# linjieli222/HERO

Hardware: AMD Instinct MI355X
Metric: videos/sec training step, HERO-base TVR-shaped batch (higher is better)
Workload: dtype bf16; 1 GPU; configs[1]: HERO-base TVR finetune micro-step (train-tvr-8gpu.json shapes: 32 videos x 60 frames, 15 subs x (4 frames + 20 tokens), 15-token query; vfeat 4352; fwd + VSM loss + bwd, all-reduce/clip/AdamW every 2nd micro-step); global_batch=32, parallelism=dp1, grad_accum=2, launch=hipGraph replay, input=one batch resident in HBM

## Files before the change

### hero_amd/_lib.py

```python
import ctypes as C
import os

import torch

_HERE = os.path.dirname(os.path.abspath(__file__))
LIB_PATH = os.environ.get("HERO_HIP_LIB") or os.path.join(_HERE, "libhero_hip.so")

ABI_VERSION = 3
F32, BF16 = 0, 1
LAYOUT_K, LAYOUT_O = 0, 1
ACT_NONE, ACT_GELU, ACT_RELU, ACT_GELU_BWD, ACT_RELU_BWD, ACT_GELU_DG, ACT_MUL_AUX = 0, 1, 2, 3, 4, 5, 6

EXPORTS = [
    "hero_last_error", "hero_abi_version", "hero_abi_struct_count", "hero_abi_struct_bytes", "hero_gemm", "hero_gemm_splits", "hero_fold_slabs", "hero_wgrad_group", "hero_wgrad_batch_plan", "hero_wgrad_batch", "hero_prof_enable", "hero_prof_read", "hero_probe_mfma", "hero_probe_hbm", "hero_gemm_force_config", "hero_layernorm_fwd",
    "hero_layernorm_bwd_workspace_bytes", "hero_layernorm_bwd", "hero_colsum_workspace_bytes",
    "hero_colsum", "hero_colsum_multi", "hero_colsum_multi_workspace_bytes", "hero_layernorm_bwd_blocks", "hero_attention_fwd", "hero_attention_bwd", "hero_attention_max_len", "hero_attention_max_packed_len", "hero_attention_stats_ok", "hero_attention_force_ppw",
    "hero_gather_rows", "hero_inverse_first", "hero_csr_gather_sum", "hero_scatter_add_rows", "hero_segment_sort_workspace_bytes", "hero_scatter_add_sorted_workspace_bytes", "hero_segment_sort", "hero_scatter_add_sorted", "hero_cast", "hero_transpose_cast", "hero_copy_multi",
    "hero_relu_bwd", "hero_gelu_bwd", "hero_add", "hero_sumsq", "hero_adamw", "hero_adamw_multi", "hero_adamw_multi_chunk",
    "hero_query_pool_fwd", "hero_query_pool_bwd", "hero_rownorm_fwd", "hero_rownorm_bwd", "hero_score_max_fwd",
    "hero_score_max_bwd", "hero_rank_loss", "hero_sums_scaled", "hero_st_ed_fwd", "hero_st_ed_bwd", "hero_st_ed_bwd_workspace_bytes",
    "hero_cross_entropy_fwd", "hero_cross_entropy_bwd", "hero_qa_pool_fwd", "hero_qa_pool_bwd",
    "hero_topk_rows", "hero_st_ed_probs", "hero_moment_topk", "hero_moment_nms", "hero_first_hit",
    "hero_collate_subs", "hero_collate_clip_mask", "hero_collate_frame_map", "hero_collate_gather_feats", "hero_derive_multi",
    "hero_comm_available", "hero_comm_unique_id", "hero_comm_init", "hero_comm_destroy", "hero_comm_rank", "hero_comm_world",
    "hero_comm_allreduce_buckets", "hero_comm_broadcast", "hero_comm_allgather", "hero_comm_allgather_var",
]


class Dropout(C.Structure):
    _fields_ = [("seed_ptr", C.c_void_p), ("site", C.c_uint64),
                ("threshold16", C.c_uint32), ("scale", C.c_float)]


class GemmEpilogue(C.Structure):
    _fields_ = [("bias", C.c_void_p), ("residual", C.c_void_p), ("aux", C.c_void_p),
                ("act", C.c_int), ("out_f32", C.c_int), ("beta", C.c_float),
                ("split_k", C.c_int), ("dropout", Dropout), ("colsum", C.c_void_p), ("colsum_partial", C.c_int), ("pad_", C.c_int), ("split_stride", C.c_longlong)]
# ... 142 lines not shown
        if have != ABI_VERSION:
            raise RuntimeError("hero_amd: %s reports ABI version %d, this binding was written against %d (struct layouts "
                               "differ: rebuild with `python -m hero_amd.build --force`)" % (LIB_PATH, have, ABI_VERSION))
        L.hero_abi_struct_bytes.argtypes = [C.c_int]
        if L.hero_abi_struct_count() != len(ABI_STRUCTS):
            raise RuntimeError("hero_amd: %s declares %d ABI structs, this binding mirrors %d" % (LIB_PATH, L.hero_abi_struct_count(), len(ABI_STRUCTS)))
        bad = [(st.__name__, C.sizeof(st), L.hero_abi_struct_bytes(i)) for i, st in enumerate(ABI_STRUCTS)
               if C.sizeof(st) != L.hero_abi_struct_bytes(i)]
        if bad:
            raise RuntimeError("hero_amd: struct layouts differ from %s (name, binding bytes, library bytes): %s" % (LIB_PATH, bad))
        L.hero_layernorm_bwd_workspace_bytes.restype = C.c_size_t
        L.hero_colsum_workspace_bytes.restype = C.c_size_t
        L.hero_colsum_multi_workspace_bytes.restype = C.c_size_t
        L.hero_colsum_multi_workspace_bytes.argtypes = [C.POINTER(Colsum), C.c_int]
        L.hero_colsum_multi.argtypes = [C.POINTER(Colsum), C.c_int, C.c_void_p, C.c_void_p]
        L.hero_layernorm_bwd_blocks.argtypes = [C.c_int]
        L.hero_gemm.argtypes = [C.c_void_p, C.c_void_p, C.c_void_p] + [C.c_int] * 9 + [
            C.POINTER(GemmEpilogue), C.c_void_p]
        L.hero_gemm_splits.argtypes = [C.c_int, C.c_int, C.c_int]
        L.hero_fold_slabs.argtypes = [C.c_void_p, C.c_int, C.c_size_t, C.c_void_p, C.c_size_t, C.c_int, C.c_void_p]
        L.hero_wgrad_group.argtypes = [C.POINTER(WgradProblem), C.c_int, C.c_int, C.c_int, C.c_void_p]
        L.hero_wgrad_batch_plan.argtypes = [C.POINTER(WgradProblem), C.c_int, C.c_int, C.c_void_p, C.c_int]
        L.hero_wgrad_batch.argtypes = [C.POINTER(WgradProblem), C.c_int, C.c_int, C.c_int, C.c_void_p, C.c_int, C.c_void_p]
        L.hero_prof_enable.argtypes = [C.c_int]
        L.hero_prof_read.argtypes = [C.c_int, C.POINTER(C.c_double), C.POINTER(C.c_double),
                                     C.POINTER(C.c_longlong)]
        L.hero_probe_mfma.argtypes = [C.c_void_p, C.c_size_t, C.POINTER(C.c_double), C.POINTER(C.c_double), C.c_void_p]
        L.hero_probe_hbm.argtypes = [C.c_void_p, C.c_void_p, C.c_size_t, C.POINTER(C.c_double), C.POINTER(C.c_double), C.c_void_p]
        L.hero_layernorm_fwd.argtypes = [C.POINTER(LnFwd), C.c_void_p]
        L.hero_layernorm_bwd.argtypes = [C.POINTER(LnBwd), C.c_void_p]
        L.hero_layernorm_bwd_workspace_bytes.argtypes = [C.c_int, C.c_int]
        L.hero_colsum_workspace_bytes.argtypes = [C.c_int, C.c_int]
        L.hero_colsum.argtypes = [C.c_void_p, C.c_void_p, C.c_int, C.c_int, C.c_int, C.c_int,
                                  C.c_float, C.c_void_p, C.c_void_p]
        L.hero_attention_fwd.argtypes = [C.POINTER(Attn), C.c_void_p]
        L.hero_attention_bwd.argtypes = [C.POINTER(Attn), C.c_void_p]
        L.hero_attention_stats_ok.argtypes = [C.c_int, C.c_int]
        L.hero_attention_force_ppw.argtypes = [C.c_int]
        L.hero_attention_max_len.argtypes = [C.c_int, C.c_int]
        L.hero_attention_max_packed_len.argtypes = [C.c_int]
        L.hero_gather_rows.argtypes = [C.c_void_p, C.c_void_p, C.c_void_p, C.c_void_p,
                                       C.c_int, C.c_int, C.c_int, C.c_void_p]
        L.hero_inverse_first.argtypes = [C.c_void_p, C.c_int, C.c_void_p, C.c_int, C.c_int, C.c_void_p]
        L.hero_csr_gather_sum.argtypes = [C.c_void_p, C.c_void_p, C.c_void_p, C.c_void_p,
                                          C.c_int, C.c_int, C.c_int, C.c_void_p]
        L.hero_scatter_add_rows.argtypes = [C.c_void_p, C.c_void_p, C.c_void_p, C.c_void_p,
# ... 91 lines not shown
```

### hero_amd/csrc/gemm_ws.hip

```cpp
#include <stdlib.h>
#include <type_traits>

#include "gemm_ws_common.h"

namespace hero {
namespace ws {

template <int TM, int TN, bool TR, int EK>
__global__ __launch_bounds__(512) __attribute__((amdgpu_waves_per_eu(2, 2))) void gemm_ws_kernel(WsArgs g) {
  typedef Geo<TM, TN> G;
  extern __shared__ __attribute__((aligned(16))) char smem[];
  const int lane = threadIdx.x & 63;
  const int wave = __builtin_amdgcn_readfirstlane(threadIdx.x >> 6);
  const int nwg = gridDim.x;
  const int wg = xcd_order(blockIdx.x, nwg);

  if (wave >= 4) {
    Loader<G, TR, ItemSource<G>> ld(ItemSource<G>{g, wg, nwg}, smem, wave - 4, lane);
    constexpr int AHEAD = (G::NSG - 2) * G::PW;
    bool more = ld.issue();
#pragma unroll
    for (int k = 0; k < G::NSG - 2; ++k) more = ld.issue();
    if (more) wait_vm<AHEAD>(); else wait_vm<0>();
    __builtin_amdgcn_s_barrier();
// ... 128 lines not shown
  ml.read_first();
  [[maybe_unused]] int seg_no = 0;
  for (int pos = start; pos < end; ++seg_no) {
    const Seg sg = seg_at<G>(g, pos, end);
    WS_T(seg_no, 0, wave, lane);
    ml.zero<false>();
    ml.run<false>(sg.nk);
    pos += sg.nk;
    WS_T(seg_no, 1, wave, lane);
#ifdef HERO_WS_TRACE
    if (blockIdx.x == 0 && lane == 0 && seg_no < 4) g_ws_trace[(seg_no * 16 + 3) * 8 + wave] = (unsigned long long)sg.nk;
#endif
    const WsgProb& P = g.p[sg.prob];
    atomic_tile<TM, TN>(P.C, P.ldc, P.M, P.N, sg.m0 + wm * TM * 32, sg.n0 + wn * TN * 32, ml.acc, lane);
    WS_T(seg_no, 14, wave, lane);
  }
}

struct WsbProb {
  const bf16_t* A;
  const bf16_t* B;
  float* C;
  float* colsum;
  int M, N, lda, ldb, ldc, pad_;
};
struct WsbItem { int prob, m0, n0, k0, nk, order, nslices, flag; };
struct WsbArgs {
  const WsbItem* items;
  int* flags;
  int rounds, K, nprob, pad_;
  WsbProb p[HERO_WGRAD_BATCH_MAX];
};

template <typename G, bool COMPUTE>
__device__ __forceinline__ void epilogue_acc(const WsbProb& P, const WsbItem& it, int* flags, char* smem, unsigned slot,
                                             f32x16_t (*acc)[G::TN], int wave, int lane, bool want_cs = false) {
  constexpr int BN = G::BN, RPP = G::RPP, RPI = G::RPI, ITERS = G::ITERS;
  char* st = smem + slot;
  const PassLane<G> pl;
  const int tid = pl.tid, c8 = pl.c8, r0 = pl.r0;
  lane = pl.lane;
  wave = pl.wave;
  const int gn = it.n0 + c8 * 8;
  const bool col_ok = r0 < RPI && gn < P.N;
  const bool plain = it.nslices == 1;
  auto tile_row = [](int p, int row) { return PassLane<G>::tile_row(p, row); };
  const __amdgpu_buffer_rsrc_t rc = __builtin_amdgcn_make_buffer_rsrc(P.C, 0, 0x7ffffff0, 0x00020000);
  if (!plain && it.order > 0) {
    if (lane == 0)
      while (__hip_atomic_load(flags + it.flag, __ATOMIC_RELAXED, __HIP_MEMORY_SCOPE_AGENT) != it.order) __builtin_amdgcn_s_sleep(8);
  }
#pragma unroll
  for (int p = 0; p < G::PASSES; ++p) {
    u32x4_t old0[ITERS], old1[ITERS];
// ... 73 lines not shown
    __builtin_amdgcn_s_barrier();
  }
  if (!plain && tid == 0)
    __hip_atomic_store(flags + it.flag, it.order + 1 < it.nslices ? it.order + 1 : 0, __ATOMIC_RELAXED, __HIP_MEMORY_SCOPE_AGENT);
}

__device__ __forceinline__ int wsb_next_round(const WsbArgs& g, int r, int nwg, int wg) {
  while (r < g.rounds && g.items[(size_t)r * nwg + wg].nk == 0) ++r;
  return r;
}

struct PlanSource {
#ifdef HERO_WSB_NOLOADS
  static constexpr bool DMA = false;
#else
  static constexpr bool DMA = true;
#endif
  const WsbArgs& g;
  int nwg, wg, lr;
  __device__ __forceinline__ bool done() const { return lr >= g.rounds; }
  __device__ __forceinline__ Panel panel() const {
    const WsbItem it = g.items[(size_t)lr * nwg + wg];
    const WsbProb& P = g.p[it.prob];
    return Panel{P.A, P.B, P.lda, P.ldb, P.M, P.N, g.K, it.m0, it.n0, it.k0 * 64, it.nk};
  }
  __device__ __forceinline__ void advance() { lr = wsb_next_round(g, lr + 1, nwg, wg); }
};

constexpr int WSB_LAB = 0
#ifdef HERO_WSB_NOLDF
                        | LAB_NOLDF
#endif
#ifdef HERO_WSB_NOMFMA
                        | LAB_NOMFMA
#endif
#ifdef HERO_WSB_NOBAR
                        | LAB_NOBAR
#endif
    ;

__global__ __launch_bounds__(512) __attribute__((amdgpu_waves_per_eu(2, 2))) void gemm_wsb_kernel(WsbArgs g) {
  typedef Geo<3, 3> G;
  constexpr int TM = 3;
  extern __shared__ __attribute__((aligned(16))) char smem[];
  const int lane = threadIdx.x & 63;
  const int wave = __builtin_amdgcn_readfirstlane(threadIdx.x >> 6);
  const int nwg = gridDim.x;
// ... 225 lines not shown
    HERO_ENSURE_LDS(&gemm_wsg_kernel, G::LDS, "gemm_wsg_kernel");
    double flops = 0.0;
    for (int i = 0; i < n; ++i) flops += 2.0 * probs[i].M * (double)probs[i].N * K;
    void* tok = gemm_prof_begin(9, s);
    hipLaunchKernelGGL(gemm_wsg_kernel, dim3(cus), dim3(512), G::LDS, s, g);
    gemm_prof_end(tok, flops, s);
    return check_launch("hero_wgrad_group");
  }
  for (int i = 0; i < n; ++i) {
    const HeroWgradProblem& q = probs[i];
    HeroGemmEpilogue e = {};
    e.out_f32 = 1; e.beta = 1.f; e.split_k = q.split_hint > 0 ? q.split_hint : 1; e.dropout.scale = 1.f;
    const int rc = hero_gemm(q.dy, q.x, q.dw, q.M, q.N, K, q.ld_dy, q.ld_x, q.ld_dw, HERO_LAYOUT_O, HERO_LAYOUT_O, dtype, &e, stream);
    if (rc) return rc;
  }
  return HERO_OK;
}

namespace hero {
namespace ws {
__device__ int g_wsb_flags[512];
constexpr int PLAN_MAGIC = 0x57534232;
constexpr int PLAN_HDR = 8;
}
}

extern "C" int hero_wgrad_batch_plan(const HeroWgradProblem* probs, int n, int K, int32_t* plan, int capacity_words) {
  using namespace hero;
  using namespace hero::ws;
  typedef Geo<3, 3> G;
  HERO_REQUIRE(probs && n >= 1 && n <= HERO_WGRAD_BATCH_MAX, "hero_wgrad_batch_plan: 1..%d problems", HERO_WGRAD_BATCH_MAX);
  HERO_REQUIRE(K >= 1, "hero_wgrad_batch_plan: K = %d", K);
  const int nwg = num_cus(), ksteps = (K + 63) / 64;
  if (nwg % 8 != 0 || ksteps < 8) return 0;
  struct T3 { int prob, mt, nt; };
  std::vector<T3> tiles;
  for (int i = 0; i < n; ++i) {
    HERO_REQUIRE(probs[i].M > 0 && probs[i].N > 0 && probs[i].M % 8 == 0 && probs[i].N % 8 == 0, "hero_wgrad_batch_plan: bad problem %d", i);
    const int tm = (probs[i].M + G::BM - 1) / G::BM, tn = (probs[i].N + G::BN - 1) / G::BN;
    const int per = nwg / 8;
    int pm = tm < 8 ? tm : 8;
    int pn = per / pm > 0 ? per / pm : 1;
    if (pn > tn) { pn = tn; pm = per / pn < tm ? per / pn : tm; if (pm < 1) pm = 1; }
    for (int bm = 0; bm < tm; bm += pm)
      for (int bn = 0; bn < tn; bn += pn)
        for (int mi = bm; mi < bm + pm && mi < tm; ++mi)
          for (int ni = bn; ni < bn + pn && ni < tn; ++ni) tiles.push_back({i, mi, ni});
  }
  const int T = (int)tiles.size();
  const int full = T / nwg, rem = T % nwg;
  struct Piece { int slot, round, tile, k0, nk, order, nslices; };
  std::vector<Piece> pieces;
  int tail_rounds = rem ? 1 : 0, S = 1;
  const int per_xcd_cap = nwg / 8, per_xcd = rem ? (rem + 7) / 8 : 0;
  if (rem) {
    HERO_REQUIRE(per_xcd <= 512 / 8, "hero_wgrad_batch_plan: flag capacity");
    for (int xcd = 0; xcd * per_xcd < rem; ++xcd) {
      const int t0 = xcd * per_xcd, p = (rem - t0 < per_xcd) ? rem - t0 : per_xcd, c = per_xcd_cap;
      int Sx = c / p;
      while (Sx > 1 && ksteps / Sx < 4) --Sx;
      if (Sx > 8) Sx = 8;
      auto cost_us = [&](int sl) { return (double)((ksteps + sl - 1) / sl) * 1.17 + (sl == 1 ? 8.0 : 9.0 + 16.0 * sl); };
      while (Sx > 1 && cost_us(Sx - 1) <= cost_us(Sx)) --Sx;
      const int L = c - Sx * p;
      const int E = 6;
      int q = (int)(((long long)p * ksteps + (long long)(p - L) * E + c - 1) / c);
      int r = ksteps - Sx * q;
      if (L == 0 || Sx != c / p || ksteps < 128 || r * 8 < ksteps) { r = 0; q = ksteps; }
      if (xcd == 0) S = Sx;
      std::vector<std::vector<Piece>> of_tile(p);
      int slot = Sx * p, fillq = 0, rnd = 0;
// ... 14 lines not shown
        }
        int k0 = 0, ord = 0;
        for (int i = (int)mine.size() - 1; i >= 0; --i) { mine[i].k0 = k0; mine[i].order = ord++; k0 += mine[i].nk; }
        of_tile[t] = mine;
      }
      for (int t = 0; t < p; ++t) {
        const int nrem = (int)of_tile[t].size();
        const int big0 = r;
        for (int sl = 0; sl < Sx; ++sl) {
          const int k0 = big0 + (int)((long long)(ksteps - big0) * sl / Sx), k1 = big0 + (int)((long long)(ksteps - big0) * (sl + 1) / Sx);
          of_tile[t].push_back({sl * p + t, 0, t, k0, k1 - k0, nrem + sl, 0});
        }
        for (Piece& pc : of_tile[t]) {
          pc.nslices = (int)of_tile[t].size();
          pc.slot += xcd * per_xcd_cap;
          pc.tile = t0 + t;
          if (pc.round + 1 > tail_rounds) tail_rounds = pc.round + 1;
          pieces.push_back(pc);
        }
      }
    }
  }
  const int rounds = full + tail_rounds;
  const int words = PLAN_HDR + rounds * nwg * 8;
  HERO_REQUIRE(plan && capacity_words >= words, "hero_wgrad_batch_plan: needs %d words, capacity %d", words, capacity_words);
  for (int i = PLAN_HDR; i < words; ++i) plan[i] = 0;
  auto item = [&](int r, int w) { return plan + PLAN_HDR + ((size_t)r * nwg + w) * 8; };
  for (int r = 0; r < full; ++r)
    for (int w = 0; w < nwg; ++w) {
      const T3& t = tiles[(size_t)r * nwg + w];
      int32_t* q = item(r, w);
      q[0] = t.prob; q[1] = t.mt * G::BM; q[2] = t.nt * G::BN; q[3] = 0; q[4] = ksteps; q[5] = 0; q[6] = 1; q[7] = 0;
    }
  for (const Piece& pc : pieces) {
    const T3& t = tiles[(size_t)full * nwg + pc.tile];
    int32_t* q = item(full + pc.round, pc.slot);
    HERO_REQUIRE(q[4] == 0, "hero_wgrad_batch_plan: internal error (slot used twice)");
    q[0] = t.prob; q[1] = t.mt * G::BM; q[2] = t.nt * G::BN; q[3] = pc.k0; q[4] = pc.nk; q[5] = pc.order; q[6] = pc.nslices;
    q[7] = (pc.slot / per_xcd_cap) * (512 / 8) + (pc.tile % per_xcd);
  }
  plan[0] = PLAN_MAGIC; plan[1] = nwg; plan[2] = rounds; plan[3] = rounds * nwg; plan[4] = n; plan[5] = K; plan[6] = T; plan[7] = S;
  return words;
}

extern "C" int hero_wgrad_batch(const HeroWgradProblem* probs, int n, int K, int dtype, const int32_t* plan_dev, int plan_words,
                                hero_stream_t stream) {
  using namespace hero;
  using namespace hero::ws;
  typedef Geo<3, 3> G;
  HERO_REQUIRE(probs && n >= 1 && n <= HERO_WGRAD_BATCH_MAX, "hero_wgrad_batch: 1..%d problems", HERO_WGRAD_BATCH_MAX);
  HERO_REQUIRE(dtype == HERO_BF16, "hero_wgrad_batch: bf16 only (dtype %d)", dtype);
  HERO_REQUIRE(plan_dev && plan_words > PLAN_HDR && (plan_words - PLAN_HDR) % (8 * num_cus()) == 0,
               "hero_wgrad_batch: the plan (%d words) was not made for this device (%d workgroups)", plan_words, num_cus());
  HERO_REQUIRE(((uintptr_t)plan_dev & 15) == 0, "hero_wgrad_batch: plan_dev must be 16-byte aligned");
  hipStream_t s = static_cast<hipStream_t>(stream);
  WsbArgs g;
  double flops = 0.0;
  for (int i = 0; i < n; ++i) {
    const HeroWgradProblem& q = probs[i];
    HERO_REQUIRE(q.dy && q.x && q.dw && q.M > 0 && q.N > 0 && q.M % 8 == 0 && q.N % 8 == 0 && q.ld_dy % 8 == 0 && q.ld_x % 8 == 0 &&
                     q.ld_dw % 4 == 0 && (((uintptr_t)q.dy | (uintptr_t)q.x | (uintptr_t)q.dw) & 15) == 0 &&
                     (size_t)64 * q.ld_dy * 2 < 0x7fffffffull && (size_t)64 * q.ld_x * 2 < 0x7fffffffull &&
                     (size_t)q.M * q.ld_dw * 4 < 0x7ffffff0ull,
                 "hero_wgrad_batch: problem %d is unaligned / too large", i);
    WsbProb& P = g.p[i];
    P.A = static_cast<const bf16_t*>(q.dy); P.B = static_cast<const bf16_t*>(q.x); P.C = q.dw;
    P.M = q.M; P.N = q.N; P.lda = q.ld_dy; P.ldb = q.ld_x; P.ldc = q.ld_dw; P.pad_ = 0;
    P.colsum = q.dbias;
    flops += 2.0 * q.M * (double)q.N * K;
  }
  for (int i = n; i < HERO_WGRAD_BATCH_MAX; ++i) g.p[i] = g.p[0];
  g.items = reinterpret_cast<const WsbItem*>(plan_dev + PLAN_HDR);
  g.rounds = (plan_words - PLAN_HDR) / (8 * num_cus());
  g.K = K; g.nprob = n; g.pad_ = 0;
  static int* flags_of[64] = {};
  int dev = 0;
  (void)hipGetDevice(&dev);
  HERO_REQUIRE(dev >= 0 && dev < 64, "hero_wgrad_batch: device %d", dev);
  if (!flags_of[dev]) HERO_REQUIRE(hipGetSymbolAddress(reinterpret_cast<void**>(&flags_of[dev]), HIP_SYMBOL(hero::ws::g_wsb_flags)) == hipSuccess,
                                   "hero_wgrad_batch: flag storage");
  g.flags = flags_of[dev];
  HERO_ENSURE_LDS(&gemm_wsb_kernel, G::LDS, "gemm_wsb_kernel");
  void* tok = gemm_prof_begin(9, s);
  hipLaunchKernelGGL(gemm_wsb_kernel, dim3(num_cus()), dim3(512), G::LDS, s, g);
  gemm_prof_end(tok, flops, s);
  return check_launch("hero_wgrad_batch");
}
```

### hero_amd/functional.py

```python
import ctypes as C
import math
import os
import weakref

import numpy as np
import torch

from . import _lib as L

_COMPUTE_DTYPE = torch.bfloat16


def set_compute_dtype(dtype):
    global _COMPUTE_DTYPE
    if dtype not in (torch.float32, torch.bfloat16):
        raise ValueError("compute dtype must be torch.float32 or torch.bfloat16")
    _COMPUTE_DTYPE = dtype


def compute_dtype():
    return _COMPUTE_DTYPE


class _Rng:
# ... 302 lines not shown
_WQ_TASK = [-1]
GROUP_WGRADS = [True]
WGRAD_BATCH = [32]
WGRAD_DBIAS_RIDE = [True]
WGRAD_RIDE_MAX_ROWS = [1 << 30]
B1_EPILOGUE = [False]
B1_PARTIALS = [True]
WGRAD_QUEUE_BYTES = [int(os.environ.get("HERO_WGRAD_QUEUE_MB", "4096")) << 20]
_WQ_BYTES = [0]
_WPLANS = {}
_WPLANS_PINNED = set()


def _wgrad_queue_full(device):
    if _WQ_BYTES[0] <= WGRAD_QUEUE_BYTES[0]:
        return False
    hard = _WQ_HARD.get(device.index)
    if hard is None:
        env = os.environ.get("HERO_WGRAD_QUEUE_HARD_MB")
        hard = (int(env) << 20) if env else max(2 * WGRAD_QUEUE_BYTES[0], int(0.15 * torch.cuda.get_device_properties(device).total_memory))
        _WQ_HARD[device.index] = hard
    if _WQ_BYTES[0] > hard:
        return True
    tiles = sum(-(-e[4] // 192) * -(-e[1].shape[1] // 192) for e in _WQ)
    full, rem = divmod(tiles, 256)
    if rem == 0:
        return True
    p = -(-rem // 8)
    slices = max(1, min(32 // p, 8))
    return tiles / 256.0 >= 0.9 * (full + (1.4 if slices > 1 else 1.0) / slices)


_WQ_HARD = {}


def _wgrad_limit():
    return 4 if (WGRAD_BATCH[0] <= 4 or SINK.wants_overlap()) else min(WGRAD_BATCH[0], 32)


def _wgrad_plan(probs, n, rows, device):
    key = (rows, device.index, tuple((probs[i].M, probs[i].N) for i in range(n)))
    hit = _WPLANS.get(key, False)
    if hit is False:
        buf = np.zeros(8 + 8 * 512 * 16, dtype=np.int32)
        words = L.lib().hero_wgrad_batch_plan(probs, n, rows, buf.ctypes.data, buf.size)
        if words < 0:
            L.check(words)
        hit = (torch.from_numpy(buf[:words].copy()).to(device), words) if words > 0 else None
        if len(_WPLANS) > 256:
            for k in [k for k in _WPLANS if k not in _WPLANS_PINNED][:128]:
                del _WPLANS[k]
        _WPLANS[key] = hit
    if hit is not None and torch.cuda.is_current_stream_capturing():
        _WPLANS_PINNED.add(key)
    return hit


_CB_TASK = [-1]


def _ensure_flush_callback(task):
    if _CB_TASK[0] != task:
        _CB_TASK[0] = task
        torch.autograd.Variable._execution_engine.queue_callback(deferred_flush)


def deferred_flush():
    _CB_TASK[0] = -1
# ... 20 lines not shown
        colsum_flush()


def colsum_flush():
    while _CQ:
        part, seen = [], []
        while _CQ and len(part) < 64:
            lo = _CQ[0][1].dst
            hi = lo + 4 * _CQ[0][2].numel()
            if any(lo < b and a < hi for a, b in seen):
                break
            seen.append((lo, hi))
            part.append(_CQ.pop(0))
        n = len(part)
        probs = (L.Colsum * n)(*[e[1] for e in part])
        need = L.lib().hero_colsum_multi_workspace_bytes(probs, n) // 4
        ws = _workspace(max(need, 1), part[0][2].device, slot="colsum_multi")
        L.check(L.lib().hero_colsum_multi(probs, n, L.ptr(ws), L.stream()))
        for e in part:
            if e[3] is not None:
                e[3]()


def wgrad_flush():
    _WQ_BYTES[0] = 0
    while _WQ:
        rows, dtype = _WQ[0][0].shape[0], _WQ[0][0].dtype
        dst_key = lambda e: (e[2].data_ptr(), e[6].data_ptr() if e[6] is not None else None)
        seen_w, seen_b = {_WQ[0][2].data_ptr()}, {dst_key(_WQ[0])[1]} - {None}
        n = 1
        while n < len(_WQ) and n < 32 and _WQ[n][0].shape[0] == rows and _WQ[n][0].dtype == dtype:
            kw, kb = dst_key(_WQ[n])
            if kw in seen_w or (kb is not None and kb in seen_b):
                break
            seen_w.add(kw)
            if kb is not None:
                seen_b.add(kb)
            n += 1
        group, rest = _WQ[:n], _WQ[n:]
        del _WQ[:]
        _WQ.extend(rest)
        probs = (L.WgradProblem * n)()
        for i, (dy2, x2, out, col0, N, _, _, _) in enumerate(group):
            K = x2.shape[1]
            probs[i] = L.WgradProblem(L.ptr(dy2) + col0 * dy2.element_size(), L.ptr(x2), L.ptr(out), N, K,
                                      dy2.shape[1], K, K, _split_for(N, K, rows, 64 if dtype == torch.bfloat16 else 32), None)
        plan = _wgrad_plan(probs, n, rows, group[0][0].device) if dtype == torch.bfloat16 else None
        if plan is not None:
            ride = WGRAD_DBIAS_RIDE[0] and rows <= WGRAD_RIDE_MAX_ROWS[0]
            for i, e in enumerate(group):
                probs[i].dbias = L.ptr(e[6]) if ride else None
                if not ride and e[6] is not None:
                    k_colsum(e[0], out=e[6], beta=1.0, col0=e[3], ncols=e[4], on_done=lambda: None)
            L.check(L.lib().hero_wgrad_batch(probs, n, rows, L.BF16, L.ptr(plan[0]), plan[1], L.stream()))
            for e in group:
                if e[6] is not None and e[7] is not None:
                    e[7]()
        else:
            for g0 in range(0, n, 4):
                sub = (L.WgradProblem * min(4, n - g0))(*[probs[i] for i in range(g0, min(g0 + 4, n))])
                L.check(L.lib().hero_wgrad_group(sub, len(sub), rows, L.dt(group[0][0]), L.stream()))
            for dy2, _, _, col0, N, _, dbias, dbias_done in group:
                if dbias is not None:
                    k_colsum(dy2, out=dbias, beta=1.0, col0=col0, ncols=N, on_done=dbias_done or (lambda: None))
        for e in group:
            if e[5] is not None:
                e[5]()


def k_wgrad(dy2, x2, out=None, beta=0.0, col0=0, ncols=None, on_done=None, dbias=None, dbias_done=None):
    M, ld = dy2.shape
    N = ld - col0 if ncols is None else ncols
    K = x2.shape[1]
    if (out is not None and beta == 1.0 and GROUP_WGRADS[0] and out.is_contiguous() and dy2.is_contiguous()
            and x2.is_contiguous() and torch._C._current_graph_task_id() != -1):
        task = torch._C._current_graph_task_id()
        if _WQ and _WQ_TASK[0] != task:
            del _WQ[:]
            _WQ_BYTES[0] = 0
        if _WQ and (_WQ[0][0].shape[0] != M or _WQ[0][0].dtype != dy2.dtype):
            wgrad_flush()
        if not _WQ:
            _WQ_TASK[0] = task
        _ensure_flush_callback(task)
        _WQ.append((dy2, x2, out, col0, N, on_done, dbias, dbias_done))
        _WQ_BYTES[0] += dy2.numel() * dy2.element_size()
        if len(_WQ) >= _wgrad_limit() or _wgrad_queue_full(dy2.device):
            wgrad_flush()
        return out
    if dbias is not None:
        k_colsum(dy2, out=dbias, beta=1.0, col0=col0, ncols=N, on_done=dbias_done or (lambda: None))
    if out is None:
        out = torch.empty((N, K), dtype=torch.float32, device=dy2.device)
    split = _split_for(N, K, M, 64 if dy2.dtype == torch.bfloat16 else 32)
    a = L.ptr(dy2) + col0 * dy2.element_size()
    k_gemm(a, x2, out, N, K, M, ld, K, K, L.LAYOUT_O, L.LAYOUT_O, L.dt(dy2), out_f32=True,
           beta=beta, split_k=split)
    if on_done is not None:
        on_done()
    return out


_WS = {}


def _workspace(n_floats, device, slot=""):
    key = (device.type, device.index, slot)
    t = _WS.get(key)
    if t is None or t.numel() < n_floats:
        t = torch.empty((max(n_floats, 1 << 20),), dtype=torch.float32, device=device)
# ... 916 lines not shown
```

### include/hero_hip.h

```cpp
#ifndef HERO_HIP_H_
#define HERO_HIP_H_

#include <stddef.h>
#include <stdint.h>

#ifdef __cplusplus
extern "C" {
#endif

typedef void* hero_stream_t;

enum { HERO_F32 = 0, HERO_BF16 = 1 };
enum { HERO_OK = 0, HERO_ERR_ARG = -1, HERO_ERR_LAUNCH = -2, HERO_ERR_UNSUPPORTED = -3 };

const char* hero_last_error(void);
#define HERO_ABI_VERSION 3
int hero_abi_version(void);
enum { HERO_STRUCT_DROPOUT = 0, HERO_STRUCT_GEMM_EPILOGUE, HERO_STRUCT_WGRAD_PROBLEM, HERO_STRUCT_LN_FWD, HERO_STRUCT_LN_BWD,
       HERO_STRUCT_COLSUM, HERO_STRUCT_ATTN, HERO_STRUCT_ADAMW, HERO_STRUCT_TENSOR_DESC, HERO_STRUCT_ADAMW_GROUP,
       HERO_STRUCT_ADAMW_MULTI, HERO_STRUCT_COPY_DESC, HERO_STRUCT_QUERY_POOL, HERO_STRUCT_ROW_NORM, HERO_STRUCT_SCORE_MAX,
       HERO_STRUCT_RANK_LOSS, HERO_STRUCT_ST_ED, HERO_STRUCT_CROSS_ENTROPY, HERO_STRUCT_DERIVE, HERO_STRUCT_COMM_BUCKET,
       HERO_STRUCT_COUNT_ };
int hero_abi_struct_count(void);
int hero_abi_struct_bytes(int which);
// ... 28 lines not shown
  int colsum_partial;
  int pad_;
  long long split_stride;
} HeroGemmEpilogue;

int hero_gemm(const void* A, const void* B, void* C, int M, int N, int K, int lda, int ldb, int ldc,
              int a_layout, int b_layout, int dtype, const HeroGemmEpilogue* epi, hero_stream_t stream);
int hero_gemm_splits(int K, int split_k, int dtype);
int hero_fold_slabs(const float* slabs, int n_slabs, size_t stride, void* out, size_t n, int out_dtype, hero_stream_t stream);

typedef struct HeroWgradProblem {
  const void* dy;
  const void* x;
  float* dw;
  int M, N, ld_dy, ld_x, ld_dw;
  int split_hint;
  float* dbias;
} HeroWgradProblem;
int hero_wgrad_group(const HeroWgradProblem* probs, int n, int K, int dtype, hero_stream_t stream);
#define HERO_WGRAD_BATCH_MAX 32
int hero_wgrad_batch_plan(const HeroWgradProblem* probs, int n, int K, int32_t* plan, int capacity_words);
int hero_wgrad_batch(const HeroWgradProblem* probs, int n, int K, int dtype, const int32_t* plan_dev, int plan_words,
                     hero_stream_t stream);
int hero_gemm_force_config(int cfg);
int hero_prof_enable(int on);
int hero_prof_read(int slot, double* total_ms, double* total_flops, long long* launches);

int hero_probe_mfma(void* scratch, size_t scratch_bytes, double* tflops, double* ghz, hero_stream_t stream);
int hero_probe_hbm(const void* src, void* dst, size_t bytes, double* copy_gbps, double* read_gbps, hero_stream_t stream);

typedef struct HeroLnFwd {
  const void* x;
  const float* tab[3];
  const int32_t* idx[3];
  const float* gamma;
  const float* beta;
  void* y;
  void* pre;
  float* mean;
  float* rstd;
  int rows, cols;
  float eps;
  int x_dtype, y_dtype;
  HeroDropout dropout;
} HeroLnFwd;
int hero_layernorm_fwd(const HeroLnFwd* a, hero_stream_t stream);
// ... 295 lines not shown
```

Baseline: 5524 videos/s.

## Batch weight-gradient GEMMs with different row counts into one persistent launch

Extends the persistent batched wgrad kernel so each problem carries its own reduction length K. The planner schedules the longest-K problems with the existing equal-split scheme, then greedily places shorter-K tiles onto the least-loaded workgroups, favouring whichever XCD has the most such workgroups. The Python queue no longer flushes when the row count changes, so wgrads from different encoders (e.g. frame and token paths) can share one launch of up to 64 problems. This reduces launch count and tail idle time, but brings a larger kernel argument struct, more complex host planning, and a changed flush heuristic that may form groups of different sizes.

```diff
diff --git a/hero_amd/_lib.py b/hero_amd/_lib.py
--- a/hero_amd/_lib.py
+++ b/hero_amd/_lib.py
@@ -12,7 +12,7 @@
 ACT_NONE, ACT_GELU, ACT_RELU, ACT_GELU_BWD, ACT_RELU_BWD, ACT_GELU_DG, ACT_MUL_AUX = 0, 1, 2, 3, 4, 5, 6
 
 EXPORTS = [
-    "hero_last_error", "hero_abi_version", "hero_abi_struct_count", "hero_abi_struct_bytes", "hero_gemm", "hero_gemm_splits", "hero_fold_slabs", "hero_wgrad_group", "hero_wgrad_batch_plan", "hero_wgrad_batch", "hero_prof_enable", "hero_prof_read", "hero_probe_mfma", "hero_probe_hbm", "hero_gemm_force_config", "hero_layernorm_fwd",
+    "hero_last_error", "hero_abi_version", "hero_abi_struct_count", "hero_abi_struct_bytes", "hero_gemm", "hero_gemm_splits", "hero_fold_slabs", "hero_wgrad_group", "hero_wgrad_batch_plan", "hero_wgrad_batch", "hero_wgrad_batch_plan_rows", "hero_wgrad_batch_rows", "hero_prof_enable", "hero_prof_read", "hero_probe_mfma", "hero_probe_hbm", "hero_gemm_force_config", "hero_layernorm_fwd",
     "hero_layernorm_bwd_workspace_bytes", "hero_layernorm_bwd", "hero_colsum_workspace_bytes",
     "hero_colsum", "hero_colsum_multi", "hero_colsum_multi_workspace_bytes", "hero_layernorm_bwd_blocks", "hero_attention_fwd", "hero_attention_bwd", "hero_attention_max_len", "hero_attention_max_packed_len", "hero_attention_stats_ok", "hero_attention_force_ppw",
     "hero_gather_rows", "hero_inverse_first", "hero_csr_gather_sum", "hero_scatter_add_rows", "hero_segment_sort_workspace_bytes", "hero_scatter_add_sorted_workspace_bytes", "hero_segment_sort", "hero_scatter_add_sorted", "hero_cast", "hero_transpose_cast", "hero_copy_multi",
@@ -201,6 +201,8 @@
         L.hero_wgrad_group.argtypes = [C.POINTER(WgradProblem), C.c_int, C.c_int, C.c_int, C.c_void_p]
         L.hero_wgrad_batch_plan.argtypes = [C.POINTER(WgradProblem), C.c_int, C.c_int, C.c_void_p, C.c_int]
         L.hero_wgrad_batch.argtypes = [C.POINTER(WgradProblem), C.c_int, C.c_int, C.c_int, C.c_void_p, C.c_int, C.c_void_p]
+        L.hero_wgrad_batch_plan_rows.argtypes = [C.POINTER(WgradProblem), C.c_int, C.POINTER(C.c_int), C.c_void_p, C.c_int]
+        L.hero_wgrad_batch_rows.argtypes = [C.POINTER(WgradProblem), C.c_int, C.POINTER(C.c_int), C.c_int, C.c_void_p, C.c_int, C.c_void_p]
         L.hero_prof_enable.argtypes = [C.c_int]
         L.hero_prof_read.argtypes = [C.c_int, C.POINTER(C.c_double), C.POINTER(C.c_double),
                                      C.POINTER(C.c_longlong)]
diff --git a/hero_amd/csrc/gemm_ws.hip b/hero_amd/csrc/gemm_ws.hip
--- a/hero_amd/csrc/gemm_ws.hip
+++ b/hero_amd/csrc/gemm_ws.hip
@@ -174,14 +174,15 @@
   const bf16_t* B;
   float* C;
   float* colsum;
-  int M, N, lda, ldb, ldc, pad_;
+  int M, N, lda, ldb, ldc;
+  int K;
 };
 struct WsbItem { int prob, m0, n0, k0, nk, order, nslices, flag; };
 struct WsbArgs {
   const WsbItem* items;
   int* flags;
-  int rounds, K, nprob, pad_;
-  WsbProb p[HERO_WGRAD_BATCH_MAX];
+  int rounds, nprob, pad_[2];
+  WsbProb p[HERO_WGRAD_BATCH_ROWS_MAX];
 };
 
 template <typename G, bool COMPUTE>
@@ -301,7 +302,7 @@
   __device__ __forceinline__ Panel panel() const {
     const WsbItem it = g.items[(size_t)lr * nwg + wg];
     const WsbProb& P = g.p[it.prob];
-    return Panel{P.A, P.B, P.lda, P.ldb, P.M, P.N, g.K, it.m0, it.n0, it.k0 * 64, it.nk};
+    return Panel{P.A, P.B, P.lda, P.ldb, P.M, P.N, P.K, it.m0, it.n0, it.k0 * 64, it.nk};
   }
   __device__ __forceinline__ void advance() { lr = wsb_next_round(g, lr + 1, nwg, wg); }
 };
@@ -573,31 +574,27 @@
 __device__ int g_wsb_flags[512];
 constexpr int PLAN_MAGIC = 0x57534232;
 constexpr int PLAN_HDR = 8;
-}
-}
-
-extern "C" int hero_wgrad_batch_plan(const HeroWgradProblem* probs, int n, int K, int32_t* plan, int capacity_words) {
-  using namespace hero;
-  using namespace hero::ws;
+
+struct T3 { int prob, mt, nt; };
+
+static void patch_tiles(const HeroWgradProblem& q, int prob, int nwg, std::vector<T3>& tiles) {
   typedef Geo<3, 3> G;
-  HERO_REQUIRE(probs && n >= 1 && n <= HERO_WGRAD_BATCH_MAX, "hero_wgrad_batch_plan: 1..%d problems", HERO_WGRAD_BATCH_MAX);
-  HERO_REQUIRE(K >= 1, "hero_wgrad_batch_plan: K = %d", K);
-  const int nwg = num_cus(), ksteps = (K + 63) / 64;
-  if (nwg % 8 != 0 || ksteps < 8) return 0;
-  struct T3 { int prob, mt, nt; };
+  const int tm = (q.M + G::BM - 1) / G::BM, tn = (q.N + G::BN - 1) / G::BN;
+  const int per = nwg / 8;
+  int pm = tm < 8 ? tm : 8;
+  int pn = per / pm > 0 ? per / pm : 1;
+  if (pn > tn) { pn = tn; pm = per / pn < tm ? per / pn : tm; if (pm < 1) pm = 1; }
+  for (int bm = 0; bm < tm; bm += pm)
+    for (int bn = 0; bn < tn; bn += pn)
+      for (int mi = bm; mi < bm + pm && mi < tm; ++mi)
+        for (int ni = bn; ni < bn + pn && ni < tn; ++ni) tiles.push_back({prob, mi, ni});
+}
+
+static int plan_equal(const HeroWgradProblem* probs, const int* idx, int m, int K, int nwg, std::vector<int32_t>& items, int* T_out, int* S_out) {
+  typedef Geo<3, 3> G;
+  const int ksteps = (K + 63) / 64;
   std::vector<T3> tiles;
-  for (int i = 0; i < n; ++i) {
-    HERO_REQUIRE(probs[i].M > 0 && probs[i].N > 0 && probs[i].M % 8 == 0 && probs[i].N % 8 == 0, "hero_wgrad_batch_plan: bad problem %d", i);
-    const int tm = (probs[i].M + G::BM - 1) / G::BM, tn = (probs[i].N + G::BN - 1) / G::BN;
-    const int per = nwg / 8;
-    int pm = tm < 8 ? tm : 8;
-    int pn = per / pm > 0 ? per / pm : 1;
-    if (pn > tn) { pn = tn; pm = per / pn < tm ? per / pn : tm; if (pm < 1) pm = 1; }
-    for (int bm = 0; bm < tm; bm += pm)
-      for (int bn = 0; bn < tn; bn += pn)
-        for (int mi = bm; mi < bm + pm && mi < tm; ++mi)
-          for (int ni = bn; ni < bn + pn && ni < tn; ++ni) tiles.push_back({i, mi, ni});
-  }
+  for (int j = 0; j < m; ++j) patch_tiles(probs[idx[j]], idx[j], nwg, tiles);
   const int T = (int)tiles.size();
   const int full = T / nwg, rem = T % nwg;
   struct Piece { int slot, round, tile, k0, nk, order, nslices; };
@@ -658,10 +655,8 @@
     }
   }
   const int rounds = full + tail_rounds;
-  const int words = PLAN_HDR + rounds * nwg * 8;
-  HERO_REQUIRE(plan && capacity_words >= words, "hero_wgrad_batch_plan: needs %d words, capacity %d", words, capacity_words);
-  for (int i = PLAN_HDR; i < words; ++i) plan[i] = 0;
-  auto item = [&](int r, int w) { return plan + PLAN_HDR + ((size_t)r * nwg + w) * 8; };
+  items.assign((size_t)rounds * nwg * 8, 0);
+  auto item = [&](int r, int w) { return items.data() + ((size_t)r * nwg + w) * 8; };
   for (int r = 0; r < full; ++r)
     for (int w = 0; w < nwg; ++w) {
       const T3& t = tiles[(size_t)r * nwg + w];
@@ -675,50 +670,147 @@
     q[0] = t.prob; q[1] = t.mt * G::BM; q[2] = t.nt * G::BN; q[3] = pc.k0; q[4] = pc.nk; q[5] = pc.order; q[6] = pc.nslices;
     q[7] = (pc.slot / per_xcd_cap) * (512 / 8) + (pc.tile % per_xcd);
   }
-  plan[0] = PLAN_MAGIC; plan[1] = nwg; plan[2] = rounds; plan[3] = rounds * nwg; plan[4] = n; plan[5] = K; plan[6] = T; plan[7] = S;
+  *T_out = T; *S_out = S;
+  return rounds;
+}
+
+static int plan_rows(const HeroWgradProblem* probs, int n, const int* rows, int nwg, int32_t* plan, int capacity_words, const char* who) {
+  typedef Geo<3, 3> G;
+  HERO_REQUIRE(probs && rows && n >= 1 && n <= HERO_WGRAD_BATCH_ROWS_MAX, "%s: 1..%d problems", who, HERO_WGRAD_BATCH_ROWS_MAX);
+  HERO_REQUIRE(nwg >= 1, "%s: %d workgroups", who, nwg);
+  int kmax = 0;
+  for (int i = 0; i < n; ++i) {
+    HERO_REQUIRE(rows[i] >= 1, "%s: K = %d (problem %d)", who, rows[i], i);
+    if (rows[i] > kmax) kmax = rows[i];
+  }
+  if (nwg % 8 != 0 || (kmax + 63) / 64 < 8) return 0;
+  for (int i = 0; i < n; ++i)
+    HERO_REQUIRE(probs[i].M > 0 && probs[i].N > 0 && probs[i].M % 8 == 0 && probs[i].N % 8 == 0, "%s: bad problem %d", who, i);
+  std::vector<int> idx;
+  for (int i = 0; i < n; ++i)
+    if (rows[i] == kmax) idx.push_back(i);
+  std::vector<int32_t> items;
+  int T = 0, S = 1;
+  int rounds = plan_equal(probs, idx.data(), (int)idx.size(), kmax, nwg, items, &T, &S);
+  if (rounds < 0) return rounds;
+  if ((int)idx.size() < n) {
+    const int c = nwg / 8;
+    std::vector<long long> load(nwg, 0);
+    std::vector<int> next(nwg, 0);
+    for (int r = 0; r < rounds; ++r)
+      for (int w = 0; w < nwg; ++w) {
+        const int nk = items[((size_t)r * nwg + w) * 8 + 4];
+        if (nk) { load[w] += nk; next[w] = r + 1; }
+      }
+    int below = kmax;
+    for (;;) {
+      int K = 0;
+      for (int i = 0; i < n; ++i)
+        if (rows[i] < below && rows[i] > K) K = rows[i];
+      if (K == 0) break;
+      below = K;
+      const int ksteps = (K + 63) / 64;
+      std::vector<T3> tiles;
+      for (int i = 0; i < n; ++i)
+        if (rows[i] == K) patch_tiles(probs[i], i, nwg, tiles);
+      T += (int)tiles.size();
+      for (size_t t0 = 0; t0 < tiles.size();) {
+        int wmin = 0;
+        for (int w = 1; w < nwg; ++w)
+          if (load[w] < load[wmin]) wmin = w;
+        int best = -1, best_cnt = 0;
+        for (int x = 0; x < 8; ++x) {
+          int cnt = 0;
+          for (int w = x * c; w < (x + 1) * c; ++w) cnt += load[w] == load[wmin];
+          if (cnt > best_cnt) { best = x; best_cnt = cnt; }
+        }
+        const long long lv = load[wmin];
+        for (int w = best * c; w < (best + 1) * c && t0 < tiles.size(); ++w) {
+          if (load[w] != lv) continue;
+          if (next[w] == rounds) { ++rounds; items.resize((size_t)rounds * nwg * 8, 0); }
+          const T3& t = tiles[t0++];
+          int32_t* q = items.data() + ((size_t)next[w] * nwg + w) * 8;
+          HERO_REQUIRE(q[4] == 0, "%s: internal error (slot used twice)", who);
+          q[0] = t.prob; q[1] = t.mt * G::BM; q[2] = t.nt * G::BN; q[3] = 0; q[4] = ksteps; q[5] = 0; q[6] = 1; q[7] = 0;
+          load[w] += ksteps; ++next[w];
+        }
+      }
+    }
+  }
+  const int words = PLAN_HDR + rounds * nwg * 8;
+  HERO_REQUIRE(plan && capacity_words >= words, "%s: needs %d words, capacity %d", who, words, capacity_words);
+  for (int i = PLAN_HDR; i < words; ++i) plan[i] = items[i - PLAN_HDR];
+  plan[0] = PLAN_MAGIC; plan[1] = nwg; plan[2] = rounds; plan[3] = rounds * nwg; plan[4] = n; plan[5] = kmax; plan[6] = T; plan[7] = S;
   return words;
 }
 
-extern "C" int hero_wgrad_batch(const HeroWgradProblem* probs, int n, int K, int dtype, const int32_t* plan_dev, int plan_words,
-                                hero_stream_t stream) {
-  using namespace hero;
-  using namespace hero::ws;
+static int launch_rows(const HeroWgradProblem* probs, int n, const int* rows, int dtype, const int32_t* plan_dev, int plan_words,
+                       hero_stream_t stream, const char* who) {
   typedef Geo<3, 3> G;
-  HERO_REQUIRE(probs && n >= 1 && n <= HERO_WGRAD_BATCH_MAX, "hero_wgrad_batch: 1..%d problems", HERO_WGRAD_BATCH_MAX);
-  HERO_REQUIRE(dtype == HERO_BF16, "hero_wgrad_batch: bf16 only (dtype %d)", dtype);
+  HERO_REQUIRE(probs && rows && n >= 1 && n <= HERO_WGRAD_BATCH_ROWS_MAX, "%s: 1..%d problems", who, HERO_WGRAD_BATCH_ROWS_MAX);
+  HERO_REQUIRE(dtype == HERO_BF16, "%s: bf16 only (dtype %d)", who, dtype);
   HERO_REQUIRE(plan_dev && plan_words > PLAN_HDR && (plan_words - PLAN_HDR) % (8 * num_cus()) == 0,
-               "hero_wgrad_batch: the plan (%d words) was not made for this device (%d workgroups)", plan_words, num_cus());
-  HERO_REQUIRE(((uintptr_t)plan_dev & 15) == 0, "hero_wgrad_batch: plan_dev must be 16-byte aligned");
+               "%s: the plan (%d words) was not made for this device (%d workgroups)", who, plan_words, num_cus());
+  HERO_REQUIRE(((uintptr_t)plan_dev & 15) == 0, "%s: plan_dev must be 16-byte aligned", who);
   hipStream_t s = static_cast<hipStream_t>(stream);
   WsbArgs g;
   double flops = 0.0;
   for (int i = 0; i < n; ++i) {
     const HeroWgradProblem& q = probs[i];
+    HERO_REQUIRE(rows[i] >= 1, "%s: K = %d (problem %d)", who, rows[i], i);
     HERO_REQUIRE(q.dy && q.x && q.dw && q.M > 0 && q.N > 0 && q.M % 8 == 0 && q.N % 8 == 0 && q.ld_dy % 8 == 0 && q.ld_x % 8 == 0 &&
                      q.ld_dw % 4 == 0 && (((uintptr_t)q.dy | (uintptr_t)q.x | (uintptr_t)q.dw) & 15) == 0 &&
                      (size_t)64 * q.ld_dy * 2 < 0x7fffffffull && (size_t)64 * q.ld_x * 2 < 0x7fffffffull &&
                      (size_t)q.M * q.ld_dw * 4 < 0x7ffffff0ull,
-                 "hero_wgrad_batch: problem %d is unaligned / too large", i);
+                 "%s: problem %d is unaligned / too large", who, i);
     WsbProb& P = g.p[i];
     P.A = static_cast<const bf16_t*>(q.dy); P.B = static_cast<const bf16_t*>(q.x); P.C = q.dw;
-    P.M = q.M; P.N = q.N; P.lda = q.ld_dy; P.ldb = q.ld_x; P.ldc = q.ld_dw; P.pad_ = 0;
+    P.M = q.M; P.N = q.N; P.lda = q.ld_dy; P.ldb = q.ld_x; P.ldc = q.ld_dw; P.K = rows[i];
     P.colsum = q.dbias;
-    flops += 2.0 * q.M * (double)q.N * K;
-  }
-  for (int i = n; i < HERO_WGRAD_BATCH_MAX; ++i) g.p[i] = g.p[0];
+    flops += 2.0 * q.M * (double)q.N * rows[i];
+  }
+  for (int i = n; i < HERO_WGRAD_BATCH_ROWS_MAX; ++i) g.p[i] = g.p[0];
   g.items = reinterpret_cast<const WsbItem*>(plan_dev + PLAN_HDR);
   g.rounds = (plan_words - PLAN_HDR) / (8 * num_cus());
-  g.K = K; g.nprob = n; g.pad_ = 0;
+  g.nprob = n; g.pad_[0] = g.pad_[1] = 0;
   static int* flags_of[64] = {};
   int dev = 0;
   (void)hipGetDevice(&dev);
-  HERO_REQUIRE(dev >= 0 && dev < 64, "hero_wgrad_batch: device %d", dev);
+  HERO_REQUIRE(dev >= 0 && dev < 64, "%s: device %d", who, dev);
   if (!flags_of[dev]) HERO_REQUIRE(hipGetSymbolAddress(reinterpret_cast<void**>(&flags_of[dev]), HIP_SYMBOL(hero::ws::g_wsb_flags)) == hipSuccess,
-                                   "hero_wgrad_batch: flag storage");
+                                   "%s: flag storage", who);
   g.flags = flags_of[dev];
   HERO_ENSURE_LDS(&gemm_wsb_kernel, G::LDS, "gemm_wsb_kernel");
   void* tok = gemm_prof_begin(9, s);
   hipLaunchKernelGGL(gemm_wsb_kernel, dim3(num_cus()), dim3(512), G::LDS, s, g);
   gemm_prof_end(tok, flops, s);
-  return check_launch("hero_wgrad_batch");
-}
+  return check_launch(who);
+}
+}
+}
+
+extern "C" int hero_wgrad_batch_plan_rows(const HeroWgradProblem* probs, int n, const int* rows, int32_t* plan, int capacity_words) {
+  return hero::ws::plan_rows(probs, n, rows, hero::num_cus(), plan, capacity_words, "hero_wgrad_batch_plan_rows");
+}
+
+extern "C" int hero_wgrad_batch_plan(const HeroWgradProblem* probs, int n, int K, int32_t* plan, int capacity_words) {
+  using namespace hero;
+  HERO_REQUIRE(probs && n >= 1 && n <= HERO_WGRAD_BATCH_MAX, "hero_wgrad_batch_plan: 1..%d problems", HERO_WGRAD_BATCH_MAX);
+  int rows[HERO_WGRAD_BATCH_MAX];
+  for (int i = 0; i < n; ++i) rows[i] = K;
+  return ws::plan_rows(probs, n, rows, num_cus(), plan, capacity_words, "hero_wgrad_batch_plan");
+}
+
+extern "C" int hero_wgrad_batch_rows(const HeroWgradProblem* probs, int n, const int* rows, int dtype, const int32_t* plan_dev,
+                                     int plan_words, hero_stream_t stream) {
+  return hero::ws::launch_rows(probs, n, rows, dtype, plan_dev, plan_words, stream, "hero_wgrad_batch_rows");
+}
+
+extern "C" int hero_wgrad_batch(const HeroWgradProblem* probs, int n, int K, int dtype, const int32_t* plan_dev, int plan_words,
+                                hero_stream_t stream) {
+  using namespace hero;
+  HERO_REQUIRE(probs && n >= 1 && n <= HERO_WGRAD_BATCH_MAX, "hero_wgrad_batch: 1..%d problems", HERO_WGRAD_BATCH_MAX);
+  int rows[HERO_WGRAD_BATCH_MAX];
+  for (int i = 0; i < n; ++i) rows[i] = K;
+  return ws::launch_rows(probs, n, rows, dtype, plan_dev, plan_words, stream, "hero_wgrad_batch");
+}
diff --git a/hero_amd/functional.py b/hero_amd/functional.py
--- a/hero_amd/functional.py
+++ b/hero_amd/functional.py
@@ -348,13 +348,15 @@
         _WQ_HARD[device.index] = hard
     if _WQ_BYTES[0] > hard:
         return True
-    tiles = sum(-(-e[4] // 192) * -(-e[1].shape[1] // 192) for e in _WQ)
+    kmax = max(e[1].shape[0] for e in _WQ)
+    tiles = sum(-(-e[4] // 192) * -(-e[1].shape[1] // 192) for e in _WQ if e[1].shape[0] == kmax)
+    short = sum(-(-e[4] // 192) * -(-e[1].shape[1] // 192) * -(-e[1].shape[0] // 64) for e in _WQ if e[1].shape[0] != kmax) / float(-(-kmax // 64))
     full, rem = divmod(tiles, 256)
     if rem == 0:
         return True
     p = -(-rem // 8)
     slices = max(1, min(32 // p, 8))
-    return tiles / 256.0 >= 0.9 * (full + (1.4 if slices > 1 else 1.0) / slices)
+    return (tiles + short) / 256.0 >= 0.9 * (full + (1.4 if slices > 1 else 1.0) / slices + short / 256.0)
 
 
 _WQ_HARD = {}
@@ -364,12 +366,21 @@
     return 4 if (WGRAD_BATCH[0] <= 4 or SINK.wants_overlap()) else min(WGRAD_BATCH[0], 32)
 
 
+WGRAD_LAUNCH_MAX = 64
+
+
+def _wgrad_count_full(rows):
+    lim = _wgrad_limit()
+    return sum(1 for e in _WQ if e[1].shape[0] == rows) >= lim or len(_WQ) >= max(lim, WGRAD_LAUNCH_MAX)
+
+
 def _wgrad_plan(probs, n, rows, device):
+    rows = (rows,) * n if isinstance(rows, int) else tuple(rows)
     key = (rows, device.index, tuple((probs[i].M, probs[i].N) for i in range(n)))
     hit = _WPLANS.get(key, False)
     if hit is False:
         buf = np.zeros(8 + 8 * 512 * 16, dtype=np.int32)
-        words = L.lib().hero_wgrad_batch_plan(probs, n, rows, buf.ctypes.data, buf.size)
+        words = L.lib().hero_wgrad_batch_plan_rows(probs, n, (C.c_int * n)(*rows), buf.ctypes.data, buf.size)
         if words < 0:
             L.check(words)
         hit = (torch.from_numpy(buf[:words].copy()).to(device), words) if words > 0 else None
@@ -436,44 +447,58 @@
                 e[3]()
 
 
+def _wgrad_take(same_rows):
+    rows, dtype = _WQ[0][0].shape[0], _WQ[0][0].dtype
+    mixed = dtype == torch.bfloat16 and not same_rows and not SINK.wants_overlap()
+    dst_key = lambda e: (e[2].data_ptr(), e[6].data_ptr() if e[6] is not None else None)
+    seen_w, seen_b = {_WQ[0][2].data_ptr()}, {dst_key(_WQ[0])[1]} - {None}
+    n, count = 1, {rows: 1}
+    while n < len(_WQ) and n < (WGRAD_LAUNCH_MAX if mixed else 32) and (mixed or _WQ[n][0].shape[0] == rows) and _WQ[n][0].dtype == dtype:
+        kw, kb = dst_key(_WQ[n])
+        if kw in seen_w or (kb is not None and kb in seen_b) or count.get(_WQ[n][0].shape[0], 0) >= 32:
+            break
+        count[_WQ[n][0].shape[0]] = count.get(_WQ[n][0].shape[0], 0) + 1
+        seen_w.add(kw)
+        if kb is not None:
+            seen_b.add(kb)
+        n += 1
+    group = _WQ[:n]
+    del _WQ[:n]
+    return group
+
+
 def wgrad_flush():
     _WQ_BYTES[0] = 0
+    same_rows = False
     while _WQ:
-        rows, dtype = _WQ[0][0].shape[0], _WQ[0][0].dtype
-        dst_key = lambda e: (e[2].data_ptr(), e[6].data_ptr() if e[6] is not None else None)
-        seen_w, seen_b = {_WQ[0][2].data_ptr()}, {dst_key(_WQ[0])[1]} - {None}
-        n = 1
-        while n < len(_WQ) and n < 32 and _WQ[n][0].shape[0] == rows and _WQ[n][0].dtype == dtype:
-            kw, kb = dst_key(_WQ[n])
-            if kw in seen_w or (kb is not None and kb in seen_b):
-                break
-            seen_w.add(kw)
-            if kb is not None:
-                seen_b.add(kb)
-            n += 1
-        group, rest = _WQ[:n], _WQ[n:]
-        del _WQ[:]
-        _WQ.extend(rest)
+        group = sorted(_wgrad_take(same_rows), key=lambda e: -e[0].shape[0])
+        n, dtype = len(group), group[0][0].dtype
+        rows = tuple(e[0].shape[0] for e in group)
         probs = (L.WgradProblem * n)()
         for i, (dy2, x2, out, col0, N, _, _, _) in enumerate(group):
             K = x2.shape[1]
             probs[i] = L.WgradProblem(L.ptr(dy2) + col0 * dy2.element_size(), L.ptr(x2), L.ptr(out), N, K,
-                                      dy2.shape[1], K, K, _split_for(N, K, rows, 64 if dtype == torch.bfloat16 else 32), None)
+                                      dy2.shape[1], K, K, _split_for(N, K, rows[i], 64 if dtype == torch.bfloat16 else 32), None)
         plan = _wgrad_plan(probs, n, rows, group[0][0].device) if dtype == torch.bfloat16 else None
+        if plan is None and rows[0] != rows[-1]:
+            _WQ[:0] = group
+            same_rows = True
+            continue
+        same_rows = False
         if plan is not None:
-            ride = WGRAD_DBIAS_RIDE[0] and rows <= WGRAD_RIDE_MAX_ROWS[0]
             for i, e in enumerate(group):
+                ride = WGRAD_DBIAS_RIDE[0] and rows[i] <= WGRAD_RIDE_MAX_ROWS[0]
                 probs[i].dbias = L.ptr(e[6]) if ride else None
                 if not ride and e[6] is not None:
                     k_colsum(e[0], out=e[6], beta=1.0, col0=e[3], ncols=e[4], on_done=lambda: None)
-            L.check(L.lib().hero_wgrad_batch(probs, n, rows, L.BF16, L.ptr(plan[0]), plan[1], L.stream()))
+            L.check(L.lib().hero_wgrad_batch_rows(probs, n, (C.c_int * n)(*rows), L.BF16, L.ptr(plan[0]), plan[1], L.stream()))
             for e in group:
                 if e[6] is not None and e[7] is not None:
                     e[7]()
         else:
             for g0 in range(0, n, 4):
                 sub = (L.WgradProblem * min(4, n - g0))(*[probs[i] for i in range(g0, min(g0 + 4, n))])
-                L.check(L.lib().hero_wgrad_group(sub, len(sub), rows, L.dt(group[0][0]), L.stream()))
+                L.check(L.lib().hero_wgrad_group(sub, len(sub), rows[0], L.dt(group[0][0]), L.stream()))
             for dy2, _, _, col0, N, _, dbias, dbias_done in group:
                 if dbias is not None:
                     k_colsum(dy2, out=dbias, beta=1.0, col0=col0, ncols=N, on_done=dbias_done or (lambda: None))
@@ -492,14 +517,15 @@
         if _WQ and _WQ_TASK[0] != task:
             del _WQ[:]
             _WQ_BYTES[0] = 0
-        if _WQ and (_WQ[0][0].shape[0] != M or _WQ[0][0].dtype != dy2.dtype):
+        if _WQ and (_WQ[0][0].dtype != dy2.dtype
+                    or (_WQ[0][0].shape[0] != M and (dy2.dtype != torch.bfloat16 or SINK.wants_overlap()))):
             wgrad_flush()
         if not _WQ:
             _WQ_TASK[0] = task
         _ensure_flush_callback(task)
         _WQ.append((dy2, x2, out, col0, N, on_done, dbias, dbias_done))
         _WQ_BYTES[0] += dy2.numel() * dy2.element_size()
-        if len(_WQ) >= _wgrad_limit() or _wgrad_queue_full(dy2.device):
+        if _wgrad_count_full(M) or _wgrad_queue_full(dy2.device):
             wgrad_flush()
         return out
     if dbias is not None:
diff --git a/include/hero_hip.h b/include/hero_hip.h
--- a/include/hero_hip.h
+++ b/include/hero_hip.h
@@ -74,6 +74,10 @@
 int hero_wgrad_batch_plan(const HeroWgradProblem* probs, int n, int K, int32_t* plan, int capacity_words);
 int hero_wgrad_batch(const HeroWgradProblem* probs, int n, int K, int dtype, const int32_t* plan_dev, int plan_words,
                      hero_stream_t stream);
+#define HERO_WGRAD_BATCH_ROWS_MAX 64
+int hero_wgrad_batch_plan_rows(const HeroWgradProblem* probs, int n, const int* rows, int32_t* plan, int capacity_words);
+int hero_wgrad_batch_rows(const HeroWgradProblem* probs, int n, const int* rows, int dtype, const int32_t* plan_dev,
+                          int plan_words, hero_stream_t stream);
 int hero_gemm_force_config(int cfg);
 int hero_prof_enable(int on);
 int hero_prof_read(int slot, double* total_ms, double* total_flops, long long* launches);
```

After: 5573 videos/s, median of 6. About the same (+0.9%).
